# pairlab/SlotFormer

Hardware: AMD Instinct MI355X
Metric: rollout frames/sec at B=32, 128x128, 7 slots, 6+50 steps (SAVi-encode + SlotFormer rollout) (higher is better)
Workload: dtype f32 storage; matmul/conv on split-bf16 MFMA (bf16x3: hi*hi+hi*lo+lo*hi, f32 accumulate)

## Files before the change

### slotformer_amd/csrc/engine.hip

```cpp
#include "../../include/slotformer_hip.h"
#include "sf_internal.h"
#include <map>
#include <vector>
#include "layer_fused.h"
#include "slot_chain.h"
#include <stdlib.h>

namespace {

inline size_t pad256(size_t nfloat) { return ((nfloat * sizeof(float)) + 255) & ~(size_t)255; }

struct Bump {
  char* p;
  size_t left;
  bool ok = true;
  size_t used = 0;
  float* take(size_t nfloat) {
    const size_t bytes = pad256(nfloat);
    if (bytes > left) {
      ok = false;
      return nullptr;
    }
    float* r = p ? (float*)(p + used) : nullptr;
    used += bytes;
// ... 45 lines not shown
    } else {
      SF_TRY(sf_linear_ex(ws.x2, rd, w.lin1_w, w.lin1_b, w.norm2_g, w.norm2_b, eps, nullptr, rd, 0, ws.hid,
                          sf_rows(ffn), Mq, ffn, d, 1, st));
      SF_TRY(sf_linear_ex(ws.hid, sf_rows(ffn), w.lin2_w, w.lin2_b, nullptr, nullptr, eps, ws.x2, rd, 0, dst, rd,
                          Mq, d, ffn, 0, st));
    }
    *out = dst;
  } else {
    if (Lq != L) return sf_set_err(-1, "row pruning requires norm_first", __FILE__, __LINE__);
    int fused = 1;
    if (sf_get_precision() >= 1 && !plain_gemms(sf_thread_opts()))
      fused = sf_qkv_attn_ex(x, nullptr, nullptr, eps, w.in_proj_w, w.in_proj_b, ws.att, B, L, L, d, heads, st);
    if (fused < 0 || fused > 1) return fused;
    if (fused == 1) {
      SF_TRY(sf_linear_ex(x, rd, w.in_proj_w, w.in_proj_b, nullptr, nullptr, eps, nullptr, rd, 0, ws.qkv,
                          sf_rows(3 * d), M, 3 * d, d, 0, st));
      SF_TRY(sf_mha_ex(ws.qkv, ws.att, B, L, L, d, heads, st));
    }
    SF_TRY(sf_linear_ex(ws.att, rd, w.out_proj_w, w.out_proj_b, nullptr, nullptr, eps, x, rd, 0, ws.y, rd, M, d,
                        d, 0, st));
    SF_TRY(sf_layernorm_ex(ws.y, rd, w.norm1_g, w.norm1_b, ws.x2, rd, M, d, eps, st));
    SF_TRY(sf_linear_ex(ws.x2, rd, w.lin1_w, w.lin1_b, nullptr, nullptr, eps, nullptr, rd, 0, ws.hid,
                        sf_rows(ffn), M, ffn, d, 1, st));
    SF_TRY(sf_linear_ex(ws.hid, sf_rows(ffn), w.lin2_w, w.lin2_b, nullptr, nullptr, eps, ws.x2, rd, 0, ws.y, rd,
                        M, d, ffn, 0, st));
    SF_TRY(sf_layernorm_ex(ws.y, rd, w.norm2_g, w.norm2_b, x, rd, M, d, eps, st));
    *out = x;
  }
  return 0;
}

int check_layers(const sf_tfm_layer* l, int n) {
  if (n > 0 && !l) return -1;
  for (int i = 0; i < n; ++i) {
    const sf_tfm_layer& w = l[i];
    if (!w.norm1_g || !w.norm1_b || !w.in_proj_w || !w.in_proj_b || !w.out_proj_w || !w.out_proj_b ||
        !w.norm2_g || !w.norm2_b || !w.lin1_w || !w.lin1_b || !w.lin2_w || !w.lin2_b)
      return -1;
  }
  return 0;
}

void step_window(const sf_rollouter* m, int s, int& nf, int& f0) {
  nf = (m->single_step && s + 1 < m->window_len) ? s + 1 : m->window_len;
  f0 = m->single_step ? s + 1 - nf : s;
}

struct RolloutPlan {
  enum Path { GENERIC, LONG_WINDOW, FUSED_ROWS, FUSED_RING } path = GENERIC;
  int tok_layers = 0;
  enum Attn { HEAD_PAIRS, ALL_HEADS, ROW_TILES } attn = HEAD_PAIRS;
  enum Ffn { CHUNK_PARTS, TILE, TILE_QKV } ffn = CHUNK_PARTS;
  bool seam = false;
  bool fused() const { return path == FUSED_ROWS || path == FUSED_RING; }
};

RolloutPlan plan_rollout(const sf_rollouter* m, int B, const SfThreadOpts& o) {
  RolloutPlan p;
  if (!m || !m->layers) return p;
  const int N = m->num_slots, W = m->window_len, Lmax = W * N, nl = m->num_layers, d = m->d_model;
  bool packed = true, tok_packed = nl >= 2;
  for (int l = 0; l < nl; ++l) {
    const sf_tfm_layer& w = m->layers[l];
    packed = packed && w.lin1_packed && w.lin2_packed && w.attn_in_packed && w.attn_out_packed;
    if (l + 1 < nl) tok_packed = tok_packed && w.tok_packed;
  }
  const int precision = o.precision >= 0 ? o.precision : sf_get_precision();
  const bool fusable = packed && !plain_gemms(o) && precision >= 1 && m->norm_first;
  const bool tok_on = tok_packed && (o.layer_tok > 0 || (o.layer_tok == 0 && sf_get_layer_tok() != 0));
  if (fusable && sf_layer_fused_ok(d, m->num_heads, m->ffn_dim, Lmax)) {
    p.path = (m->in_proj_packed && m->out_proj_packed && sf_step_boundary_ok(d, m->slot_size)) ? RolloutPlan::FUSED_RING
                                                                                               : RolloutPlan::FUSED_ROWS;
    bool tok = tok_on;
    for (int nf = m->single_step ? 1 : W; nf <= W && tok; ++nf) tok = sf_layer_tok_ok(nf * N);
    p.tok_layers = tok ? nl - 1 : 0;
    p.attn = (o.attn_rows == 128 || tok) ? RolloutPlan::ROW_TILES : (o.attn_heads == 8 ? RolloutPlan::ALL_HEADS : RolloutPlan::HEAD_PAIRS);
    if (p.attn != RolloutPlan::HEAD_PAIRS && o.ffn_tile >= 1)
      p.ffn = (p.attn == RolloutPlan::ROW_TILES && o.ffn_tile == 2) ? RolloutPlan::TILE_QKV : RolloutPlan::TILE;
    const int cus = o.cus > 0 && o.cus < 160 ? o.cus : 160;
    p.seam = p.path == RolloutPlan::FUSED_RING && p.attn == RolloutPlan::HEAD_PAIRS &&
             (o.seam >= 0 ? o.seam != 0 : sf_get_seam_fused() != 0) && sf_seam_blocks(B, N) <= cus;
  } else if (fusable && sf_layer_fused_ok(d, m->num_heads, m->ffn_dim, 1) && Lmax > 64 && sf_ffn_tiles(B * Lmax) <= 1024) {
    p.path = RolloutPlan::LONG_WINDOW;
    if (tok_on && Lmax <= 96 && !m->single_step && sf_layer_tok_ok(Lmax)) p.tok_layers = nl - 1;
  }
  return p;
}

struct RolloutWs {
  float* x;
  TfmWs tw;
  float* apb;
  float* xpb;
  float *xa, *xb2;
  int* counters;
  unsigned* seam_flags;
  float* ring;
  float* planes;
};

bool rollout_ws_take(Bump& bp, RolloutWs& w, const sf_rollouter* m, int B) {
  const size_t M = (size_t)B * m->window_len * m->num_slots, d = m->d_model;
  w.x = bp.take(M * d);
  tfm_ws_take(bp, w.tw, (int)M, (int)d, m->ffn_dim);
  w.apb = bp.take(8 * M * d);
  w.xpb = bp.take(4 * M * d);
  w.xa = bp.take(M * d);
  w.xb2 = bp.take(M * d);
  w.counters = (int*)bp.take(1024);
  w.seam_flags = (unsigned*)bp.take(1024);
  w.ring = bp.take((size_t)B * (m->window_len + 1) * m->num_slots * d);
  w.planes = bp.take(sf_attn_rows_plane_bytes(B) / 4);
  return bp.ok;
}

}

extern "C" {

size_t sf_rollout_workspace_bytes(const sf_rollouter* m, int B) {
  if (!m || B <= 0) return 0;
  Bump bp{nullptr, ~(size_t)0};
  RolloutWs w;
  rollout_ws_take(bp, w, m, B);
  return bp.used;
}

__global__ void spin_kernel(long long ticks) {
  const long long t0 = wall_clock64();
  while (wall_clock64() - t0 < ticks) __builtin_amdgcn_s_sleep(16);
}
extern "C" int sf_debug_spin(int us, void* stream) {
  SF_REQUIRE(us > 0 && us <= 100000, "sf_debug_spin: 1..100000 microseconds");
  hipLaunchKernelGGL(spin_kernel, dim3(1), dim3(64), 0, (hipStream_t)stream, (long long)us * 100);
// ... 22 lines not shown
}

__global__ void zero_f32_kernel(float* a, float* b, long long n) {
  const long long i = 4 * ((long long)blockIdx.x * blockDim.x + threadIdx.x);
  if (i >= n) return;
  const bool vec = i + 4 <= n && ((((unsigned long long)(a + i)) | ((unsigned long long)(b + i))) & 15ull) == 0;
  if (vec) {
    *(float4*)(a + i) = float4{0.f, 0.f, 0.f, 0.f};
    *(float4*)(b + i) = float4{0.f, 0.f, 0.f, 0.f};
  } else {
    for (long long j = i; j < n && j < i + 4; ++j) {
      a[j] = 0.f;
      b[j] = 0.f;
    }
  }
}

__global__ void zero_words_kernel(unsigned* a, unsigned* b) {
  unsigned* p = blockIdx.x == 0 ? a : b;
  if (p) p[threadIdx.x] = 0u;
}

int sf_rollout_f32(const sf_rollouter* m, float* slots, int B, int T_total, int pred_len, void* ws,
                   size_t ws_bytes, void* stream) {
  SF_REQUIRE(m && slots && ws, "null pointer");
  SF_REQUIRE(B >= 1 && pred_len >= 0, "bad batch / pred_len");
  SF_REQUIRE(m->num_slots >= 1 && m->slot_size > 0 && (m->slot_size % 4) == 0 && m->d_model > 0 &&
                 (m->d_model % 4) == 0 && m->ffn_dim > 0 && (m->ffn_dim % 4) == 0 && m->num_layers >= 1 &&
                 m->window_len >= 1, "bad rollouter shape");
  SF_REQUIRE(m->in_proj_w && m->in_proj_b && m->out_proj_w && m->out_proj_b && m->pe_tok, "null weight");
  SF_REQUIRE(check_layers(m->layers, m->num_layers) == 0, "null transformer-layer weight");
  const int n_in = m->single_step ? 1 : m->window_len;
  SF_REQUIRE(T_total >= n_in + pred_len, "slots buffer shorter than burn-in + pred_len");
  SF_REQUIRE(ws_bytes >= sf_rollout_workspace_bytes(m, B), "workspace too small");
  hipStream_t st = (hipStream_t)stream;
  const int N = m->num_slots, C = m->slot_size, d = m->d_model, W = m->window_len, nl = m->num_layers;
  const float eps = 1e-5f;
  Bump bp{(char*)ws, ws_bytes};
  RolloutWs w;
  if (!rollout_ws_take(bp, w, m, B)) return sf_set_err(-1, "workspace too small", __FILE__, __LINE__);
  const RolloutPlan p = plan_rollout(m, B, sf_thread_opts());
  const bool ring_in = p.path == RolloutPlan::FUSED_RING;
  const bool long_ffn = p.path == RolloutPlan::LONG_WINDOW;
  const int np = p.attn == RolloutPlan::HEAD_PAIRS ? 4 : 1;
  const int RF = W + 1;
  const long long bs = (long long)T_total * N * C;
  if (ring_in) {
    SF_TRY(sf_ring_init_ex(m->out_proj_packed, m->out_proj_b, m->in_proj_packed, m->in_proj_b, slots, bs, n_in, w.ring, RF, N, B, st));
  }
  if (p.fused() || long_ffn) {
    SF_REQUIRE(sf_ffn_tiles(B * W * N) <= 1024, "batch too large for the fused-layer tile counters");
    hipLaunchKernelGGL(zero_words_kernel, dim3(2), dim3(1024), 0, st, (unsigned*)w.counters, p.seam ? w.seam_flags : nullptr);
    SF_CHECK_LAUNCH();
    if (p.attn == RolloutPlan::ROW_TILES) {
      const long long nfl = (long long)(sf_attn_rows_plane_bytes(B) / 4), half = nfl / 2;
      hipLaunchKernelGGL(zero_f32_kernel, dim3((unsigned)(((half + 3) / 4 + 255) / 256)), dim3(256), 0, st, w.planes, w.planes + half, half);
      SF_CHECK_LAUNCH();
    }
  }
  float* apb2 = w.apb + (size_t)4 * B * W * N * d;
  float* ap0 = w.apb;
  bool attn0_done = false;
  for (int s = 0; s < pred_len; ++s) {
    int nf, f0;
    step_window(m, s, nf, f0);
    const int L = nf * N, pe_off = (W - nf) * N;
    const float* pe = m->pe_tok + (long long)pe_off * d;
    float* cin = nullptr;
    if (!ring_in) {
      SfRowMap pmap = sf_rows(d);
      pmap.base = (long long)pe_off * d;
      SF_TRY(sf_linear_ex(slots, sf_rows_batched(C, L, bs, (long long)f0 * N * C), m->in_proj_w, m->in_proj_b,
                          nullptr, nullptr, 0.f, m->pe_tok, pmap, L, w.x, sf_rows(d), B * L, d, C, 0, st));
      cin = w.x;
    }
    int l = 0;
    while (l < p.tok_layers) {
      const int nlt = (p.tok_layers - l) < 8 ? (p.tok_layers - l) : 8;
      float* xo = (cin == w.xa) ? w.xb2 : w.xa;
      if (ring_in)
        SF_TRY(sf_layer_tok_ex(l == 0 ? 1 : 0, cin, w.ring, RF, N, f0, pe, m->layers + l, nlt, eps, xo, B, L, st));
      else
        SF_TRY(sf_layer_tok_ex(0, cin, nullptr, 1, 1, 0, nullptr, m->layers + l, nlt, eps, xo, B, L, st));
      cin = xo;
      l += nlt;
    }
    if (!p.fused()) {
      int Lc = L;
      for (; l < nl; ++l) {
        const int Lq = (l == nl - 1 && m->norm_first) ? N : Lc;
        SF_TRY(tfm_layer(m->layers[l], cin, w.tw, B, Lc, Lq, d, m->num_heads, m->ffn_dim, m->norm_first, st, &cin,
                         long_ffn ? w.xpb : nullptr, long_ffn ? w.counters : nullptr));
        Lc = Lq;
      }
      const SfRowMap lastmap = (Lc == N) ? sf_rows(d) : sf_rows_batched(d, N, (long long)Lc * d, (long long)(Lc - N) * d);
      SF_TRY(sf_linear_ex(cin, lastmap, m->out_proj_w, m->out_proj_b, nullptr, nullptr, 0.f, nullptr, sf_rows(C), 0,
                          slots, sf_rows_batched(C, N, bs, (long long)(n_in + s) * N * C), B * N, C, d, 0, st));
      continue;
    }
    bool parts_in = false;
    float* parked = nullptr;
    for (; l < nl; ++l) {
      const sf_tfm_layer& lw = m->layers[l];
      const bool lastl = (l == nl - 1);
      const int Lq = lastl ? N : L;
      const long long pst = (long long)B * Lq * d;
      float* xo = (cin == w.xa) ? w.xb2 : w.xa;
      float* ap = (l == 0) ? ap0 : w.apb;
      if (parked) {
        ap = parked;
        SF_TRY(sf_attn_core_ex(lw, ap, w.planes, B, L, Lq, st));
      } else if (p.attn == RolloutPlan::ROW_TILES) {
        if (l == 0 && ring_in)
          SF_TRY(sf_attn_rows_ex(2, w.ring, (long long)RF * N * d, 0, pe, f0, RF, N, lw, eps, ap, w.planes, B, L, Lq, st));
        else if (parts_in)
          SF_TRY(sf_attn_rows_ex(1, w.xpb, (long long)L * d, (long long)B * L * d, nullptr, 0, 1, 1, lw, eps, ap, w.planes, B, L, Lq, st));
        else
          SF_TRY(sf_attn_rows_ex(0, cin, (long long)L * d, 0, nullptr, 0, 1, 1, lw, eps, ap, w.planes, B, L, Lq, st));
      } else if (p.attn == RolloutPlan::ALL_HEADS) {
        if (l == 0 && ring_in)
          SF_TRY(sf_attn_all_ring_ex(w.ring, RF, N, f0, pe, lw, eps, ap, B, L, Lq, st));
        else if (parts_in)
          SF_TRY(sf_attn_all_parts_ex(w.xpb, (long long)B * L * d, lw, eps, ap, B, L, Lq, st));
        else
          SF_TRY(sf_attn_all_ex(cin, lw, eps, ap, B, L, Lq, st));
      } else if (l == 0 && ring_in) {
        if (!attn0_done) SF_TRY(sf_attn_oproj_ring_ex(w.ring, RF, N, f0, pe, lw, eps, ap, pst, B, L, Lq, st));
      } else if (parts_in) {
        SF_TRY(sf_attn_oproj_parts_ex(w.xpb, (long long)B * L * d, lw, eps, ap, pst, B, L, Lq, st));
      } else {
        SF_TRY(sf_attn_oproj_ex(cin, lw, eps, ap, pst, B, L, Lq, st));
      }
      if (!lastl) {
        if (p.ffn == RolloutPlan::TILE_QKV) {
          float* park = (ap == w.apb) ? apb2 : w.apb;
          SF_TRY(sf_ffn_qkv_tile_ex(ap, lw, m->layers[l + 1], eps, park, w.planes, B, L, (l + 1 == nl - 1) ? N : L, m->ffn_dim, st));
          parked = park;
          cin = nullptr;
        } else if (p.ffn == RolloutPlan::TILE) {
// ... 790 lines not shown
```

### slotformer_amd/csrc/layer_fused.h

```cpp
#pragma once
#include "../../include/slotformer_hip.h"
#include "sf_internal.h"

int sf_pred_step_ex(const float* prev, const sf_tfm_layer* layers, int nlayers, int heads, int ffn, int norm_first, const void* const* packed,
                    const float* lstm_b_ih, const float* lstm_b_hh, const float* proj_b, int hidden, float* lstm_h, float* lstm_c,
                    float* out, int B, int N, int D, float eps, hipStream_t st);

int sf_attn_oproj_ex(const float* xin, const sf_tfm_layer& w, float eps, float* ap, long long ap_stride, int B, int L,
                     int Lq, hipStream_t st);
int sf_attn_oproj_parts_ex(const float* xparts, long long xparts_stride, const sf_tfm_layer& w, float eps, float* ap,
                           long long ap_stride, int B, int L, int Lq, hipStream_t st);
int sf_ffn_parts_ex(const float* ap, long long ap_stride, const sf_tfm_layer& w, float eps, float* xp, long long xp_stride, int M,
                    int ffn, hipStream_t st, int np = 4);
int sf_attn_all_ex(const float* xin, const sf_tfm_layer& w, float eps, float* x2, int B, int L, int Lq, hipStream_t st);
int sf_attn_all_parts_ex(const float* xparts, long long xparts_stride, const sf_tfm_layer& w, float eps, float* x2, int B, int L,
                         int Lq, hipStream_t st);
int sf_attn_all_ring_ex(const float* ring, int ring_frames, int nslots, int f0, const float* pe, const sf_tfm_layer& w, float eps,
                        float* x2, int B, int L, int Lq, hipStream_t st);
int sf_attn_core_ex(const sf_tfm_layer& w, float* x2, void* planes, int B, int L, int Lq, hipStream_t st);
int sf_ffn_qkv_tile_ex(const float* x2, const sf_tfm_layer& w, const sf_tfm_layer& wn, float eps, float* xpark, void* planes, int B, int L, int Lq,
                       int ffn, hipStream_t st);
int sf_ffn_tile_ex(const float* x2, const sf_tfm_layer& w, float eps, float* y, int M, int ffn, hipStream_t st);
bool sf_layer_tok_ok(int L);
int sf_layer_tok_vpw(int L);
int sf_layer_tok_ex(int mode, const float* xin, const float* ring, int ring_frames, int nslots, int f0, const float* pe, const sf_tfm_layer* layers, int nl,
                    float eps, float* y, int B, int L, hipStream_t st);
size_t sf_attn_rows_plane_bytes(int B);
int sf_attn_rows_ex(int mode, const float* xin, long long x_batch_stride, long long xparts_stride, const float* pe, int f0,
                    int ring_frames, int nslots, const sf_tfm_layer& w, float eps, float* x2, void* planes, int B, int L, int Lq,
                    hipStream_t st);
int sf_attn_oproj_ring_ex(const float* ring, int ring_frames, int nslots, int f0, const float* pe, const sf_tfm_layer& w,
                          float eps, float* ap, long long ap_stride, int B, int L, int Lq, hipStream_t st);
bool sf_step_boundary_ok(int d, int slot_size);
int sf_ffn_partial_ex(const float* ap, long long ap_stride, const sf_tfm_layer& w, float eps, float* xp,
                      long long xp_stride, float* xout, int* counters, int M, int ffn, hipStream_t st, int np = 4);
int sf_ffn_tiles(int M);
int sf_ring_init_ex(const void* wout_packed, const float* b_out, const void* win_packed, const float* b_in, float* slots,
                    long long slots_bs, int n_frames, float* ring, int ring_frames, int nslots, int B, hipStream_t st);
int sf_ffn_boundary_ex(const float* ap, long long ap_stride, const sf_tfm_layer& w, float eps, float* xp, long long xp_stride,
                       int* counters, int ffn, const void* wout_packed, const float* b_out, const void* win_packed,
                       const float* b_in, float* slots, long long slots_bs, int frame, float* ring, int ring_frames, int nslots,
                       int B, hipStream_t st, int np = 4);
int sf_seam_ex(const float* ap_ffn, long long pst_ffn, const sf_tfm_layer& wl, float eps, float* xp, long long xp_stride,
               int* counters, int ffn, const void* wout_packed, const float* b_out, const void* win_packed, const float* b_in,
               float* slots, long long slots_bs, int frame, float* ring, int ring_frames, int nslots, int B,
               const sf_tfm_layer& w0, int f0_next, const float* pe, float* ap_attn, long long pst_attn, int L, int Lq,
               unsigned* seam_flags, unsigned epoch, hipStream_t st);
int sf_seam_blocks(int B, int nslots);
bool sf_seam_window_ok(int L, int nslots);
```

### slotformer_amd/csrc/layer_tok.hip

```cpp
#include "../../include/slotformer_hip.h"
#include "sf_internal.h"
#include "layer_fused.h"
#include <stdlib.h>

typedef float f32x16 __attribute__((ext_vector_type(16)));
typedef float f32x4 __attribute__((ext_vector_type(4)));
typedef __bf16 bf16x4 __attribute__((ext_vector_type(4)));
typedef __bf16 bf16x8 __attribute__((ext_vector_type(8)));

namespace {
constexpr int LT_NT = 256, LT_D = 256, LT_F = 1024, LT_NH = 8, LT_TOK = 128, LT_MAXL = 8;
constexpr int LT_STAGE = 32 * 1024, LT_RING = 3;
constexpr int LT_NST_ATT = 4 * LT_NH, LT_NST = LT_NST_ATT + 2 * (LT_F / 32);
constexpr int LT_KV = LT_RING * LT_STAGE;
constexpr int LT_VT = LT_KV + 16 * 1024;
constexpr int LT_PAR = LT_KV + 32 * 1024;
constexpr int P_LN1G = 0, P_LN1B = 256, P_BQKV = 512, P_BO = 1280, P_LN2G = 1536, P_LN2B = 1792, P_B1 = 2048, P_B2 = 3072, P_N = 3328;
constexpr size_t LT_LDS = (size_t)LT_PAR + (size_t)P_N * 4;
constexpr size_t LT_BLOB = (size_t)LT_NST * LT_STAGE + (size_t)P_N * 4;
static_assert(LT_LDS <= 160 * 1024, "LDS budget");

struct LtArgs {
  const float* x;
  const float* ring;
  const float* pe;
  float* y;
  const char* blob[LT_MAXL];
  float eps;
  int nl, B, L, vpw, RF, N, f0, dbg_ts;
};

__device__ __forceinline__ bf16x8 cat8(bf16x4 a, bf16x4 b) { return __builtin_shufflevector(a, b, 0, 1, 2, 3, 4, 5, 6, 7); }
__device__ __forceinline__ void split8(const f32x4 a, const f32x4 b, bf16x8& hi, bf16x8& lo) {
  const bf16x4 h0 = __builtin_convertvector(a, bf16x4), h1 = __builtin_convertvector(b, bf16x4);
  const bf16x4 l0 = __builtin_convertvector(a - __builtin_convertvector(h0, f32x4), bf16x4);
  const bf16x4 l1 = __builtin_convertvector(b - __builtin_convertvector(h1, f32x4), bf16x4);
  hi = cat8(h0, h1);
  lo = cat8(l0, l1);
}
__device__ __forceinline__ f32x4 quad(const f32x16& a, int g) { return f32x4{a[4 * g], a[4 * g + 1], a[4 * g + 2], a[4 * g + 3]}; }
__device__ __forceinline__ float lt_xother(float v, int h) {
#ifdef LT_SHFL
  return __shfl_xor(v, 32, 64);
#endif
  const unsigned u = __builtin_bit_cast(unsigned, v);
  const auto r = __builtin_amdgcn_permlane32_swap(u, u, false, false);
  return __builtin_bit_cast(float, h ? r[0] : r[1]);
}
__device__ __forceinline__ float lt_xmax(float v, int h) { return fmaxf(v, lt_xother(v, h)); }
__device__ __forceinline__ float lt_xsum(float v, int h) {
  const float o = lt_xother(v, h);
  return h ? o + v : v + o;
}

struct LtRing {
  const char* rd;
  const char* src;
  char* dst;
};
__device__ __forceinline__ void lt_dma_now(const LtRing& R, int f) {
  __builtin_amdgcn_global_load_lds((const void __attribute__((address_space(1)))*)(R.src + f * 1024),
                                   (void __attribute__((address_space(3)))*)(R.dst + f * 1024), 16, 0, 0);
}
__device__ __forceinline__ void lt_dma(const LtRing& R, int f) {
#if defined(LT_NODMA) || defined(LT_BURST)
  return;
#endif
#ifndef LT_NOIMMOFF
  const void __attribute__((address_space(1)))* s = (const void __attribute__((address_space(1)))*)(R.src + (f >> 2) * 4096);
  void __attribute__((address_space(3)))* d = (void __attribute__((address_space(3)))*)(R.dst + (f >> 2) * 4096);
  switch (f & 3) {
    case 0: __builtin_amdgcn_global_load_lds(s, d, 16, 0, 0); break;
    case 1: __builtin_amdgcn_global_load_lds(s, d, 16, 1024, 0); break;
    case 2: __builtin_amdgcn_global_load_lds(s, d, 16, 2048, 0); break;
    default: __builtin_amdgcn_global_load_lds(s, d, 16, 3072, 0); break;
  }
#else
  __builtin_amdgcn_global_load_lds((const void __attribute__((address_space(1)))*)(R.src + f * 1024),
                                   (void __attribute__((address_space(3)))*)(R.dst + f * 1024), 16, 0, 0);
#endif
}
#define LT_MFMA(a, b, c) __builtin_amdgcn_mfma_f32_32x32x16_bf16(a, b, c, 0, 0, 0)
// ... 212 lines not shown
      hd = 7; kind = 3;
    } else {
      const int tq = st - 3;
      kind = tq & 3;
      hd = 1 + (tq >> 2) - (kind == 3 ? 1 : 0);
    }
    slice = kind == 3;
    ld = LT_D;
    if (!slice) {
      W = win; r0 = (kind == 0 ? 0 : kind == 1 ? 256 : 512) + 32 * hd;
    } else {
      W = wout; c0 = 32 * hd;
    }
  } else {
    const int ff = st - LT_NST_ATT;
    int hb;
    if (ff == 0) {
      slice = false; hb = 0;
    } else if (ff == 63) {
      slice = true; hb = 31;
    } else if (ff & 1) {
      slice = false; hb = (ff + 1) >> 1;
    } else {
      slice = true; hb = (ff >> 1) - 1;
    }
    if (!slice) {
      W = w1; ld = LT_D; r0 = 32 * hb;
    } else {
      W = w2; ld = LT_F; c0 = 32 * hb;
    }
  }
  if (!slice) {
    const int vk = f >> 1;
    c0 = 32 * (vk >> 1);
    s = vk & 1;
  } else {
    r0 = 32 * (f >> 2);
    s = (f >> 1) & 1;
  }
  const float* src = W + (long long)(r0 + i) * ld + c0 + 4 * h;
  union {
    __bf16 b[8];
    uint4 u;
  } o;
#pragma unroll
  for (int j = 0; j < 8; ++j) {
    const float v = src[8 * (2 * s + (j >> 2)) + (j & 3)];
    const __bf16 hi = (__bf16)v;
    o.b[j] = pl ? (__bf16)(v - (float)hi) : hi;
  }
  out[idx] = o.u;
}

__device__ long long lt_ts[16];
#define LTS(i) do { if (A.dbg_ts && blockIdx.x == 0 && threadIdx.x == 0) lt_ts[i] = wall_clock64(); } while (0)

template <int MODE>
__global__ __launch_bounds__(LT_NT) void layer_tok_kernel(LtArgs A) {
  extern __shared__ __attribute__((aligned(16))) char smem[];
  float* P = (float*)(smem + LT_PAR);
  const int t = threadIdx.x, lane = t & 63;
  const int wave = __builtin_amdgcn_readfirstlane(t >> 6);
  const int n = lane & 31, h = lane >> 5;
  const int L = A.L;
  const int v0 = blockIdx.x * A.vpw;
  const int nvalid = min(A.vpw, A.B - v0) * L;
  const int tl = wave * 32 + n;
  const int te = min(tl, nvalid - 1);
  const int vl = te / L, tok = te - vl * L;
  const long long row = (long long)(v0 + vl) * L + tok;
  LTS(0);
  f32x16 X[8];
  if constexpr (MODE == 0) {
    const float* xr = A.x + row * LT_D + 4 * h;
#pragma unroll
    for (int ob = 0; ob < 8; ++ob)
#pragma unroll
      for (int g = 0; g < 4; ++g) {
        const f32x4 v = *(const f32x4*)(xr + 32 * ob + 8 * g);
#pragma unroll
        for (int q = 0; q < 4; ++q) X[ob][4 * g + q] = v[q];
      }
  } else {
    const int fr = tok / A.N, sl = tok - fr * A.N;
    const float* rr = A.ring + (((long long)(v0 + vl) * A.RF + (A.f0 + fr) % A.RF) * A.N + sl) * LT_D + 4 * h;
    const float* pr = A.pe + (long long)tok * LT_D + 4 * h;
#pragma unroll
    for (int ob = 0; ob < 8; ++ob)
#pragma unroll
      for (int g = 0; g < 4; ++g) {
        const f32x4 v = *(const f32x4*)(rr + 32 * ob + 8 * g);
#pragma unroll
        for (int q = 0; q < 4; ++q) X[ob][4 * g + q] = v[q];
      }
    __builtin_amdgcn_sched_barrier(0);
#pragma unroll
    for (int ob = 0; ob < 8; ++ob) {
#pragma unroll
      for (int g = 0; g < 4; ++g) {
        const f32x4 v = *(const f32x4*)(pr + 32 * ob + 8 * g);
#pragma unroll
        for (int q = 0; q < 4; ++q) X[ob][4 * g + q] += v[q];
      }
      __builtin_amdgcn_sched_barrier(0);
    }
  }
  const unsigned wlane = (unsigned)(wave * 8 * 1024 + lane * 16);
  char* const wdst = smem + (wave * 8) * 1024;
  int cur = 0;
  int cs = -2;
// ... 25 lines not shown
    const long long c0 = __builtin_readcyclecounter();
    if (c_last) c_work += c0 - c_last;
#endif
#ifdef LT_NODMA
    asm volatile("s_waitcnt vmcnt(0)" ::: "memory");
#else
    asm volatile("s_waitcnt vmcnt(8)" ::: "memory");
#endif
    asm volatile("s_waitcnt lgkmcnt(0)" ::: "memory");
#ifdef LT_STAMPS
    const long long c1 = __builtin_readcyclecounter();
#endif
#ifndef LT_NOBAR
    __builtin_amdgcn_s_barrier();
#endif
    asm volatile("" ::: "memory");
#ifdef LT_STAMPS
    c_last = __builtin_readcyclecounter();
    c_wait += c1 - c0;
    c_bar += c_last - c1;
#endif
    const int nb = cur == 0 ? 2 : cur - 1;
    LtRing R{smem + cur * LT_STAGE + lane * 16, stage_src(), wdst + nb * LT_STAGE};
#ifdef LT_BURST
#pragma unroll
    for (int f = 0; f < 8; ++f) lt_dma_now(R, f);
#endif
    cur = cur == 2 ? 0 : cur + 1;
    return R;
  };
  const int wf = min(wave * 32, nvalid - 1);
  const int kb0 = ((wf / L) * L) >> 5;
  const int d0 = 32 * kb0 + 4 * h - vl * L;
  const char* pb;
  {
    unsigned pbo = (unsigned)(LT_PAR + 16 * h);
    asm volatile("" : "+v"(pbo));
    pb = smem + pbo;
  }
  char* const kwr = smem + LT_KV + wave * 1024 + lane * 16;
  char* const vwr = smem + LT_VT + wave * 4096 + lane * 16;
  const char* krd[3];
  const char* vrd[3];
#pragma unroll
  for (int kbi = 0; kbi < 3; ++kbi) {
    const int kb = min(kb0 + kbi, 3);
    krd[kbi] = smem + LT_KV + kb * 1024 + lane * 16;
    vrd[kbi] = smem + LT_VT + kb * 4096 + lane * 16;
  }
  const float qscale = 0.2550348616841918f;
  constexpr float NEG = -3.0e38f;
  LTS(1);

#pragma unroll 1
  for (int l = 0; l < A.nl; ++l) {
    cs = 0;
    base_cur = A.blob[l];
    last_layer = l + 1 >= A.nl;
    base_nxt = A.blob[last_layer ? l : l + 1];
    __syncthreads();
    {
      const float* vsrc = (const float*)(A.blob[l] + (size_t)LT_NST * LT_STAGE);
      for (int i = t; i < P_N / 4; i += LT_NT) *(f32x4*)(P + 4 * i) = *(const f32x4*)(vsrc + 4 * i);
    }
    __syncthreads();
    if (l == 0) LTS(2);
    bf16x8 xh[16], xl[16];
    lt_layernorm<P_LN1G, P_LN1B>(X, pb, h, A.eps, xh, xl);
    lt_add_vec<P_BO>(X, pb);
    if (l == 0) LTS(3);
    f32x16 qa, ka, va, S[3], O;
    bf16x8 qh[2], ql[2], ph[3][2], pl[3][2], oh[2], ol[2];
    float mx0 = NEG, mx1 = NEG, mx = 0.f, sm = 0.f, rinv = 0.f;
    auto zero16 = [](f32x16& a) {
#pragma unroll
      for (int r = 0; r < 16; ++r) a[r] = 0.f;
    };
    int hq = 0;
    auto mask_chunk = [&](int c) {
      const int kbi = c >> 1;
#pragma unroll
      for (int rr = 0; rr < 8; ++rr) {
        const int r = 8 * (c & 1) + rr;
        const bool ok = (unsigned)(d0 + 32 * kbi + 8 * (r >> 2) + (r & 3)) < (unsigned)L;
        const float v = ok ? S[kbi][r] : NEG;
        S[kbi][r] = v;
        if (rr & 1) mx1 = fmaxf(mx1, v); else mx0 = fmaxf(mx0, v);
      }
    };
    auto exp_chunk = [&](int c) {
      const int kbi = c >> 1;
      float s0 = 0.f, s1 = 0.f;
#pragma unroll
      for (int rr = 0; rr < 8; ++rr) {
        const int r = 8 * (c & 1) + rr;
#ifdef LT_EXPF
        const float e = __expf((S[kbi][r] - mx) * 0.6931471805599453f);
#else
        const float e = __builtin_amdgcn_exp2f(S[kbi][r] - mx);
#endif
        S[kbi][r] = e;
        if (rr & 1) s1 += e; else s0 += e;
      }
      sm += s0 + s1;
    };
    auto psplit_chunk = [&](int c) { split8(quad(S[c >> 1], 2 * (c & 1)), quad(S[c >> 1], 2 * (c & 1) + 1), ph[c >> 1][c & 1], pl[c >> 1][c & 1]); };
    auto kconv = [&](int s) {
      const float* bk = (const float*)pb + P_BQKV + 256 + 32 * hq;
// ... 87 lines not shown
      lt_row_product<true, 5>(R, xh, xl, va, [&](int g) {
        if (g < 2) kconv(g);
        else if (g < 4) qconv(g - 2);
      });
      vconv(0);
      vconv(1);
    }
#pragma unroll 1
    for (hq = 1; hq < LT_NH; ++hq) {
      {
        const LtRing R = stage_begin();
        scores();
          lt_row_product<false, 6>(R, xh, xl, qa, sideD);
      }
      {
        const LtRing R = stage_begin();
          lt_row_product<false, 6>(R, xh, xl, ka, sideA);
        pv();
      }
      {
        const LtRing R = stage_begin();
          lt_row_product<true, 5>(R, xh, xl, va, [&](int g) {
          if (g < 2) kconv(g);
          else if (g < 4) qconv(g - 2);
          else if (g < 6) oconv(g - 4);
        });
      }
      {
        const LtRing R = stage_begin();
        lt_kslice_product<5>(R, oh, ol, X, [&](int g) {
          if (g < 2) vconv(g);
        });
      }
    }
    asm volatile("s_waitcnt lgkmcnt(0)" ::: "memory");
    __builtin_amdgcn_s_barrier();
    asm volatile("" ::: "memory");
    scores();
#pragma unroll
    for (int g = 0; g < 8; ++g) sideD(g);
#pragma unroll
    for (int g = 0; g < 6; ++g) sideA(g);
    pv();
    oconv(0);
    oconv(1);
    {
      const LtRing R = stage_begin();
      lt_kslice_product<0>(R, oh, ol, X, LtNoSide{});
    }
    if (l == 0) LTS(4);
#ifdef LT_STAMPS
    if (l == 0 && blockIdx.x == 0 && threadIdx.x == 0) { lt_ts[8] = c_wait; lt_ts[9] = c_bar; lt_ts[10] = c_work; }
#endif
    lt_layernorm<P_LN2G, P_LN2B>(X, pb, h, A.eps, xh, xl);
    lt_add_vec<P_B2>(X, pb);
    if (l == 0) LTS(5);
    f32x16 Ha, Hb;
    bf16x8 hh[2], hl[2];
    f32x4 b1q[4];
    auto b1_load = [&](int blk) {
      const float* b1 = (const float*)pb + P_B1 + 32 * blk;
#pragma unroll
      for (int g = 0; g < 4; ++g) b1q[g] = *(const f32x4*)(b1 + 8 * g);
    };
    auto hconv = [&](const f32x16& Hx, int s) {
      const f32x4 z4 = {0.f, 0.f, 0.f, 0.f};
      const f32x4 u0 = __builtin_elementwise_max(quad(Hx, 2 * s) + b1q[2 * s], z4);
      const f32x4 u1 = __builtin_elementwise_max(quad(Hx, 2 * s + 1) + b1q[2 * s + 1], z4);
      split8(u0, u1, hh[s], hl[s]);
    };
    auto ffn_step = [&](f32x16& Hn, const f32x16& Hp, int j) {
      {
        const LtRing R = stage_begin();
        lt_row_product<false, 4>(R, xh, xl, Hn, [&](int g) {
          if (g >= 1 && g < 3) hconv(Hp, g - 1);
        });
        asm volatile("" : "+v"(hh[0]), "+v"(hh[1]), "+v"(hl[0]), "+v"(hl[1]));
      }
      {
        const LtRing R = stage_begin();
        b1_load(j);
        lt_kslice_product<0>(R, hh, hl, X, LtNoSide{});
      }
    };
    {
      const LtRing R = stage_begin();
      b1_load(0);
      lt_row_product<false, 0>(R, xh, xl, Ha, LtNoSide{});
    }
    ffn_step(Hb, Ha, 1);
#pragma unroll 1
    for (int j = 2; j < LT_F / 32; j += 2) {
      ffn_step(Ha, Hb, j);
      ffn_step(Hb, Ha, j + 1);
    }
    hconv(Hb, 0);
    hconv(Hb, 1);
    {
      const LtRing R = stage_begin();
      lt_kslice_product<0>(R, hh, hl, X, LtNoSide{});
    }
    if (l == 0) LTS(6);
#ifdef LT_STAMPS
    if (l == 0 && blockIdx.x == 0 && threadIdx.x == 0) { lt_ts[11] = c_wait; lt_ts[12] = c_bar; lt_ts[13] = c_work; }
#endif
  }
  asm volatile("s_waitcnt vmcnt(0)" ::: "memory");
  if (tl < nvalid) {
    float* yr = A.y + row * LT_D + 4 * h;
#pragma unroll
    for (int ob = 0; ob < 8; ++ob)
#pragma unroll
      for (int g = 0; g < 4; ++g) *(f32x4*)(yr + 32 * ob + 8 * g) = quad(X[ob], g);
  }
  LTS(7);
}

extern "C" int sf_debug_read_ts_layer_tok(long long* out16) {
  hipError_t e = hipMemcpyFromSymbol(out16, HIP_SYMBOL(lt_ts), sizeof(long long) * 16);
  return e == hipSuccess ? 0 : (int)e;
}

extern "C" size_t sf_layer_tok_packed_bytes(void) { return LT_BLOB; }

extern "C" int sf_pack_layer_tok_weights(const sf_tfm_layer* w, void* packed, int d_model, int num_heads, int ffn, void* stream) {
  SF_REQUIRE(w && packed, "sf_pack_layer_tok_weights: null pointer");
  SF_REQUIRE(w->in_proj_w && w->out_proj_w && w->lin1_w && w->lin2_w && w->norm1_g && w->norm1_b && w->in_proj_b && w->out_proj_b && w->norm2_g &&
                 w->norm2_b && w->lin1_b && w->lin2_b, "sf_pack_layer_tok_weights: null weight");
  SF_REQUIRE(d_model == LT_D && num_heads == LT_NH && ffn == LT_F, "sf_pack_layer_tok_weights: d_model 256, 8 heads, ffn 1024 only");
  hipStream_t st = (hipStream_t)stream;
  const int total = LT_NST * 32 * 64;
  hipLaunchKernelGGL(pack_layer_tok_kernel, dim3((total + 255) / 256), dim3(256), 0, st, w->in_proj_w, w->out_proj_w, w->lin1_w, w->lin2_w, (uint4*)packed);
  SF_CHECK_LAUNCH();
  float* vec = (float*)((char*)packed + (size_t)LT_NST * LT_STAGE);
  const struct {
    const float* src;
    int off, n;
  } parts[8] = {{w->norm1_g, P_LN1G, 256}, {w->norm1_b, P_LN1B, 256}, {w->in_proj_b, P_BQKV, 768}, {w->out_proj_b, P_BO, 256},
                {w->norm2_g, P_LN2G, 256}, {w->norm2_b, P_LN2B, 256}, {w->lin1_b, P_B1, 1024},   {w->lin2_b, P_B2, 256}};
  for (const auto& p : parts) {
    const hipError_t e = hipMemcpyAsync(vec + p.off, p.src, (size_t)p.n * 4, hipMemcpyDeviceToDevice, st);
    if (e != hipSuccess) return sf_set_err((int)e, hipGetErrorString(e), __FILE__, __LINE__);
  }
  return 0;
}

int sf_layer_tok_vpw(int L) {
  if (L < 1 || L > 96) return 0;
  for (int vpw = LT_TOK / L; vpw >= 1; --vpw) {
    const int nvalid = vpw * L;
    bool ok = true;
    for (int w = 0; w < 4 && ok; ++w) {
      const int wf = w * 32 < nvalid ? w * 32 : nvalid - 1, wl = w * 32 + 31 < nvalid ? w * 32 + 31 : nvalid - 1;
      const int kb0 = ((wf / L) * L) >> 5, kb1 = (((wl / L) * L) + L - 1) >> 5;
      ok = kb1 - kb0 + 1 <= 3;
    }
    if (ok) return vpw;
  }
  return 0;
}
bool sf_layer_tok_ok(int L) { return sf_layer_tok_vpw(L) > 0; }

int sf_layer_tok_ex(int mode, const float* xin, const float* ring, int ring_frames, int nslots, int f0, const float* pe, const sf_tfm_layer* layers, int nl,
                    float eps, float* y, int B, int L, hipStream_t st) {
  bool ok = layers && nl >= 1 && nl <= LT_MAXL && sf_layer_tok_ok(L) && B >= 1 && y && (mode == 0 ? xin != nullptr : (ring && pe && nslots >= 1 && ring_frames >= 1));
  for (int l = 0; ok && l < nl; ++l) ok = layers[l].tok_packed != nullptr;
  if (!ok)
    return sf_set_err(-1, "invalid argument: the token-stationary layers need sf_pack_layer_tok_weights fragments, 1..8 layers and 1 <= L <= 96 rows per video", __FILE__, __LINE__);
  static const int dbg = sf_dbg("lt");
  LtArgs A;
  A.x = xin; A.ring = ring; A.pe = pe; A.y = y;
  for (int l = 0; l < LT_MAXL; ++l) A.blob[l] = (const char*)layers[l < nl ? l : nl - 1].tok_packed;
  A.eps = eps; A.nl = nl; A.B = B; A.L = L; A.vpw = sf_layer_tok_vpw(L); A.RF = ring_frames; A.N = nslots; A.f0 = f0; A.dbg_ts = dbg;
  const int nwg = (B + A.vpw - 1) / A.vpw;
  const double flops = nl * ((double)B * L * (2.0 * LT_D * (3 * LT_D + LT_D + 2 * LT_F)) + (double)B * LT_NH * 4.0 * L * L * 32);
  if (mode == 0) {
    SF_TRY(sf_ensure_dyn_lds((const void*)layer_tok_kernel<0>, LT_LDS));
    sf_prof_begin(SF_K_LAYER_TOK, st, flops);
    hipLaunchKernelGGL(layer_tok_kernel<0>, dim3(nwg), dim3(LT_NT), LT_LDS, st, A);
  } else {
    SF_TRY(sf_ensure_dyn_lds((const void*)layer_tok_kernel<1>, LT_LDS));
    sf_prof_begin(SF_K_LAYER_TOK, st, flops);
    hipLaunchKernelGGL(layer_tok_kernel<1>, dim3(nwg), dim3(LT_NT), LT_LDS, st, A);
  }
  sf_prof_end(SF_K_LAYER_TOK, st);
  SF_CHECK_LAUNCH();
  return 0;
}

extern "C" int sf_layer_tok_block_f32(const sf_tfm_layer* w, int nl, const float* x, float* y, int B, int L, void* stream) {
  SF_REQUIRE(w && x && y && B > 0 && nl >= 1 && nl <= LT_MAXL, "sf_layer_tok_block_f32: null pointer / empty problem / more than 8 layers");
  SF_REQUIRE(sf_get_precision() == 1, "sf_layer_tok_block_f32: split-bf16 mode only");
  return sf_layer_tok_ex(0, x, nullptr, 1, 1, 0, nullptr, w, nl, 1e-5f, y, B, L, (hipStream_t)stream);
}
```

Measured before the change: 668,700.

## Fold last transformer layer and slot boundary projections into token-stationary kernel

Extends the token-stationary layer kernel so the final transformer layer (attention plus LN2, FFN, residual) and the out-projection and in-projection at the step boundary run inside the same launch, only for the last N slot rows. The kernel writes predicted slots and the next ring entry directly, so the per-step launches of the separate fused last-layer path and its plane zeroing are skipped. The cost is a longer kernel with FFN weights streamed per workgroup from registers and LDS. Only one wave-group of 32 rows does the tail work, which may be underutilized.

```diff
diff --git a/slotformer_amd/csrc/engine.hip b/slotformer_amd/csrc/engine.hip
--- a/slotformer_amd/csrc/engine.hip
+++ b/slotformer_amd/csrc/engine.hip
@@ -121,6 +121,7 @@
   enum Attn { HEAD_PAIRS, ALL_HEADS, ROW_TILES } attn = HEAD_PAIRS;
   enum Ffn { CHUNK_PARTS, TILE, TILE_QKV } ffn = CHUNK_PARTS;
   bool seam = false;
+  bool fold = false;
   bool fused() const { return path == FUSED_ROWS || path == FUSED_RING; }
 };
 
@@ -149,6 +150,8 @@
     const int cus = o.cus > 0 && o.cus < 160 ? o.cus : 160;
     p.seam = p.path == RolloutPlan::FUSED_RING && p.attn == RolloutPlan::HEAD_PAIRS &&
              (o.seam >= 0 ? o.seam != 0 : sf_get_seam_fused() != 0) && sf_seam_blocks(B, N) <= cus;
+    p.fold = p.path == RolloutPlan::FUSED_RING && p.tok_layers == nl - 1 && p.tok_layers > 0 && m->layers[nl - 1].tok_packed && !m->single_step &&
+             m->ffn_dim == 1024 && sf_layer_tok_fold_ok(Lmax, N);
   } else if (fusable && sf_layer_fused_ok(d, m->num_heads, m->ffn_dim, 1) && Lmax > 64 && sf_ffn_tiles(B * Lmax) <= 1024) {
     p.path = RolloutPlan::LONG_WINDOW;
     if (tok_on && Lmax <= 96 && !m->single_step && sf_layer_tok_ok(Lmax)) p.tok_layers = nl - 1;
@@ -277,7 +280,7 @@
     SF_REQUIRE(sf_ffn_tiles(B * W * N) <= 1024, "batch too large for the fused-layer tile counters");
     hipLaunchKernelGGL(zero_words_kernel, dim3(2), dim3(1024), 0, st, (unsigned*)w.counters, p.seam ? w.seam_flags : nullptr);
     SF_CHECK_LAUNCH();
-    if (p.attn == RolloutPlan::ROW_TILES) {
+    if (p.attn == RolloutPlan::ROW_TILES && !p.fold) {
       const long long nfl = (long long)(sf_attn_rows_plane_bytes(B) / 4), half = nfl / 2;
       hipLaunchKernelGGL(zero_f32_kernel, dim3((unsigned)(((half + 3) / 4 + 255) / 256)), dim3(256), 0, st, w.planes, w.planes + half, half);
       SF_CHECK_LAUNCH();
@@ -303,13 +306,18 @@
     while (l < p.tok_layers) {
       const int nlt = (p.tok_layers - l) < 8 ? (p.tok_layers - l) : 8;
       float* xo = (cin == w.xa) ? w.xb2 : w.xa;
-      if (ring_in)
-        SF_TRY(sf_layer_tok_ex(l == 0 ? 1 : 0, cin, w.ring, RF, N, f0, pe, m->layers + l, nlt, eps, xo, B, L, st));
-      else
+      if (ring_in) {
+        const SfTokFold fold{m->layers + nl - 1, m->ffn_dim, m->out_proj_packed, m->in_proj_packed, m->out_proj_b, m->in_proj_b,
+                             slots, bs, n_in + s, w.ring, RF};
+        const bool fold_here = p.fold && l + nlt == p.tok_layers;
+        SF_TRY(sf_layer_tok_ex(l == 0 ? 1 : 0, cin, w.ring, RF, N, f0, pe, m->layers + l, nlt, eps, xo, B, L, st, fold_here ? &fold : nullptr));
+      } else {
         SF_TRY(sf_layer_tok_ex(0, cin, nullptr, 1, 1, 0, nullptr, m->layers + l, nlt, eps, xo, B, L, st));
+      }
       cin = xo;
       l += nlt;
     }
+    if (p.fold) continue;
     if (!p.fused()) {
       int Lc = L;
       for (; l < nl; ++l) {
diff --git a/slotformer_amd/csrc/layer_fused.h b/slotformer_amd/csrc/layer_fused.h
--- a/slotformer_amd/csrc/layer_fused.h
+++ b/slotformer_amd/csrc/layer_fused.h
@@ -23,8 +23,20 @@
 int sf_ffn_tile_ex(const float* x2, const sf_tfm_layer& w, float eps, float* y, int M, int ffn, hipStream_t st);
 bool sf_layer_tok_ok(int L);
 int sf_layer_tok_vpw(int L);
+struct SfTokFold {
+  const sf_tfm_layer* last;
+  int ffn;
+  const void *wout_packed, *win_packed;
+  const float *b_out, *b_in;
+  float* slots;
+  long long slots_bs;
+  int frame;
+  float* ring;
+  int ring_frames;
+};
+bool sf_layer_tok_fold_ok(int L, int nslots);
 int sf_layer_tok_ex(int mode, const float* xin, const float* ring, int ring_frames, int nslots, int f0, const float* pe, const sf_tfm_layer* layers, int nl,
-                    float eps, float* y, int B, int L, hipStream_t st);
+                    float eps, float* y, int B, int L, hipStream_t st, const SfTokFold* fold = nullptr);
 size_t sf_attn_rows_plane_bytes(int B);
 int sf_attn_rows_ex(int mode, const float* xin, long long x_batch_stride, long long xparts_stride, const float* pe, int f0,
                     int ring_frames, int nslots, const sf_tfm_layer& w, float eps, float* x2, void* planes, int B, int L, int Lq,
diff --git a/slotformer_amd/csrc/layer_tok.hip b/slotformer_amd/csrc/layer_tok.hip
--- a/slotformer_amd/csrc/layer_tok.hip
+++ b/slotformer_amd/csrc/layer_tok.hip
@@ -25,9 +25,14 @@
   const float* ring;
   const float* pe;
   float* y;
-  const char* blob[LT_MAXL];
+  const char* blob[LT_MAXL + 1];
   float eps;
   int nl, B, L, vpw, RF, N, f0, dbg_ts;
+  const uint4 *w1p, *w2p, *wout_p, *win_p;
+  const float *ln2g, *ln2b, *b1, *b2, *b_out, *b_in;
+  float* slots;
+  float* ring_out;
+  long long slots_bs, slots_off, ring_bs, ring_off;
 };
 
 __device__ __forceinline__ bf16x8 cat8(bf16x4 a, bf16x4 b) { return __builtin_shufflevector(a, b, 0, 1, 2, 3, 4, 5, 6, 7); }
@@ -346,10 +351,202 @@
   out[idx] = o.u;
 }
 
+constexpr int PF_AP = LT_D + 8, PF_XP = LT_D + 4, PF_C = 128, PF_PP = PF_C + 8;
+constexpr size_t PF_AH = 0, PF_AL = PF_AH + 32 * PF_AP * 2, PF_HH = PF_AL + 32 * PF_AP * 2, PF_HL = PF_HH + 32 * PF_AP * 2;
+constexpr size_t PF_X2 = PF_HL + 32 * PF_AP * 2, PF_END = PF_X2 + (size_t)32 * PF_XP * 4;
+static_assert(PF_END <= (size_t)LT_PAR && (size_t)2 * 32 * PF_PP * 2 <= 2 * 32 * PF_AP * 2, "folded last layer: LDS budget");
+
+__device__ __forceinline__ void lt_split4(__bf16* hp, __bf16* lp, int off, f32x4 v) {
+  const bf16x4 hi = __builtin_convertvector(v, bf16x4);
+  const bf16x4 lo = __builtin_convertvector(v - __builtin_convertvector(hi, f32x4), bf16x4);
+  *(bf16x4*)(hp + off) = hi;
+  *(bf16x4*)(lp + off) = lo;
+}
+__device__ __forceinline__ f32x16 lt_frag_product(const bf16x8 (&wf)[16][2], const __bf16* bh, const __bf16* bl) {
+  f32x16 a0, a1;
+#pragma unroll
+  for (int r = 0; r < 16; ++r) a0[r] = a1[r] = 0.f;
+#pragma unroll
+  for (int ks = 0; ks < 16; ks += 2) {
+    const bf16x8 xh0 = *(const bf16x8*)(bh + ks * 16), xl0 = *(const bf16x8*)(bl + ks * 16);
+    const bf16x8 xh1 = *(const bf16x8*)(bh + ks * 16 + 16), xl1 = *(const bf16x8*)(bl + ks * 16 + 16);
+    a0 = LT_MFMA(wf[ks][0], xl0, a0);
+    a1 = LT_MFMA(wf[ks + 1][0], xl1, a1);
+    a0 = LT_MFMA(wf[ks][1], xh0, a0);
+    a1 = LT_MFMA(wf[ks + 1][1], xh1, a1);
+    a0 = LT_MFMA(wf[ks][0], xh0, a0);
+    a1 = LT_MFMA(wf[ks + 1][0], xh1, a1);
+  }
+  return a0 + a1;
+}
+
+__device__ __forceinline__ void lt_fold_tail(const LtArgs& A, char* smem, const f32x16 (&X)[8], int wave, int lane, int tl, int te, int nvalid) {
+#pragma clang fp contract(off)
+  __bf16* Ah = (__bf16*)(smem + PF_AH);
+  __bf16* Al = (__bf16*)(smem + PF_AL);
+  __bf16* Hh = (__bf16*)(smem + PF_HH);
+  __bf16* Hl = (__bf16*)(smem + PF_HL);
+  float* X2 = (float*)(smem + PF_X2);
+  const int n = lane & 31, h = lane >> 5, L = A.L, N = A.N;
+  const int v0 = blockIdx.x * A.vpw, nq = (nvalid / L) * N;
+  {
+    const int vl = te / L, tok = te - vl * L;
+    if (tl < nvalid && tok >= L - N) {
+      float* xr = X2 + (vl * N + tok - (L - N)) * PF_XP + 4 * h;
+#pragma unroll
+      for (int ob = 0; ob < 8; ++ob)
+#pragma unroll
+        for (int g = 0; g < 4; ++g) *(f32x4*)(xr + 32 * ob + 8 * g) = quad(X[ob], g);
+    }
+  }
+  __syncthreads();
+  {
+    const f32x4 g = *(const f32x4*)(A.ln2g + 4 * lane), be = *(const f32x4*)(A.ln2b + 4 * lane);
+#pragma unroll
+    for (int i = 0; i < 8; ++i) {
+      const int r = wave + 4 * i;
+      const f32x4 x2 = *(const f32x4*)(X2 + min(r, nq - 1) * PF_XP + 4 * lane);
+      const float mean = sf_sum64((x2[0] + x2[1]) + (x2[2] + x2[3])) * (1.0f / LT_D);
+      const f32x4 dv = x2 - mean;
+      const float rstd = 1.0f / sqrtf(sf_sum64((dv[0] * dv[0] + dv[1] * dv[1]) + (dv[2] * dv[2] + dv[3] * dv[3])) * (1.0f / LT_D) + A.eps);
+      lt_split4(Ah, Al, r * PF_AP + 4 * lane, (x2 - mean) * rstd * g + be);
+    }
+  }
+  __syncthreads();
+  const int ao = n * PF_AP + 8 * h;
+  const int rn = min(n, nq - 1);
+  bf16x8 wf[2][16][2];
+  auto load = [&](int j, bf16x8 (&w)[16][2]) {
+    const int c = j >> 2, wb = wave + 4 * (j & 1);
+    const uint4* base = (((j >> 1) & 1) ? A.w2p : A.w1p) + ((long long)(c * 16) * 8 + wb) * 128 + lane;
+#pragma unroll
+    for (int ks = 0; ks < 16; ++ks)
+#pragma unroll
+      for (int pl = 0; pl < 2; ++pl) w[ks][pl] = __builtin_bit_cast(bf16x8, base[(ks * 8) * 128 + pl * 64]);
+  };
+  f32x16 Hacc[2], Y[2];
+  load(0, wf[0]);
+#pragma unroll
+  for (int j = 0; j < 16; ++j) {
+    if (j + 1 < 16) load(j + 1, wf[(j + 1) & 1]);
+    const int c = j >> 2, jb = j & 1, wb = wave + 4 * jb;
+    if (((j >> 1) & 1) == 0) {
+      Hacc[jb] = lt_frag_product(wf[j & 1], Ah + ao, Al + ao);
+      if (jb == 1) {
+        __syncthreads();
+#pragma unroll
+        for (int b = 0; b < 2; ++b) {
+          const int hb = wave + 4 * b;
+#pragma unroll
+          for (int g = 0; g < 4; ++g) {
+            const f32x4 bv = *(const f32x4*)(A.b1 + c * 256 + hb * 32 + 4 * h + 8 * g);
+            f32x4 hv;
+#pragma unroll
+            for (int q = 0; q < 4; ++q) hv[q] = fmaxf(Hacc[b][4 * g + q] + bv[q], 0.f);
+            lt_split4(Hh, Hl, n * PF_AP + hb * 32 + 4 * h + 8 * g, hv);
+          }
+        }
+        __syncthreads();
+      }
+    } else {
+      const f32x16 p = lt_frag_product(wf[j & 1], Hh + ao, Hl + ao);
+      if (c == 0) {
+#pragma unroll
+        for (int g = 0; g < 4; ++g) {
+          const int col = wb * 32 + 4 * h + 8 * g;
+          const f32x4 r = *(const f32x4*)(X2 + rn * PF_XP + col) + *(const f32x4*)(A.b2 + col);
+#pragma unroll
+          for (int q = 0; q < 4; ++q) Y[jb][4 * g + q] = p[4 * g + q] + r[q];
+        }
+      } else {
+#pragma unroll
+        for (int r = 0; r < 16; ++r) Y[jb][r] = Y[jb][r] + p[r];
+      }
+    }
+  }
+#pragma unroll
+  for (int b = 0; b < 2; ++b)
+#pragma unroll
+    for (int g = 0; g < 4; ++g) lt_split4(Ah, Al, n * PF_AP + (wave + 4 * b) * 32 + 4 * h + 8 * g, quad(Y[b], g));
+  __syncthreads();
+  const bool st_ok = n < nq;
+  const long long vb = v0 + n / N, sn = n - (n / N) * N;
+  __bf16* Ph = Hh;
+  __bf16* Pl = Hh + 32 * PF_PP;
+  {
+    bf16x8 wo[16][2];
+#pragma unroll
+    for (int ks = 0; ks < 16; ++ks)
+#pragma unroll
+      for (int pl = 0; pl < 2; ++pl) wo[ks][pl] = __builtin_bit_cast(bf16x8, A.wout_p[(((long long)ks * 4 + wave) * 2 + pl) * 64 + lane]);
+    f32x16 a0, a1;
+#pragma unroll
+    for (int r = 0; r < 16; ++r) a0[r] = a1[r] = 0.f;
+#pragma unroll
+    for (int k = 0; k < 8; ++k) {
+      const bf16x8 xh0 = *(const bf16x8*)(Ah + ao + k * 16), xl0 = *(const bf16x8*)(Al + ao + k * 16);
+      const bf16x8 xh1 = *(const bf16x8*)(Ah + ao + 128 + k * 16), xl1 = *(const bf16x8*)(Al + ao + 128 + k * 16);
+      a0 = LT_MFMA(wo[k][0], xl0, a0);
+      a1 = LT_MFMA(wo[8 + k][0], xl1, a1);
+      a0 = LT_MFMA(wo[k][1], xh0, a0);
+      a1 = LT_MFMA(wo[8 + k][1], xh1, a1);
+      a0 = LT_MFMA(wo[k][0], xh0, a0);
+      a1 = LT_MFMA(wo[8 + k][0], xh1, a1);
+    }
+#pragma unroll
+    for (int g = 0; g < 4; ++g) {
+      const int col = wave * 32 + 4 * h + 8 * g;
+      const f32x4 bo = *(const f32x4*)(A.b_out + col);
+      f32x4 v;
+#pragma unroll
+      for (int q = 0; q < 4; ++q) v[q] = a0[4 * g + q] + a1[4 * g + q] + bo[q];
+      lt_split4(Ph, Pl, n * PF_PP + col, v);
+      if (st_ok) *(f32x4*)(A.slots + vb * A.slots_bs + A.slots_off + sn * PF_C + col) = v;
+    }
+  }
+  __syncthreads();
+  {
+    bf16x8 wi[2][8][2];
+#pragma unroll
+    for (int b = 0; b < 2; ++b)
+#pragma unroll
+      for (int k = 0; k < 8; ++k)
+#pragma unroll
+        for (int pl = 0; pl < 2; ++pl) wi[b][k][pl] = __builtin_bit_cast(bf16x8, A.win_p[(((long long)k * 8 + wave + 4 * b) * 2 + pl) * 64 + lane]);
+    f32x16 a[2];
+#pragma unroll
+    for (int r = 0; r < 16; ++r) a[0][r] = a[1][r] = 0.f;
+    const int po = n * PF_PP + 8 * h;
+#pragma unroll
+    for (int k = 0; k < 8; ++k) {
+      const bf16x8 xh = *(const bf16x8*)(Ph + po + k * 16), xl = *(const bf16x8*)(Pl + po + k * 16);
+#pragma unroll
+      for (int b = 0; b < 2; ++b) a[b] = LT_MFMA(wi[b][k][0], xl, a[b]);
+#pragma unroll
+      for (int b = 0; b < 2; ++b) a[b] = LT_MFMA(wi[b][k][1], xh, a[b]);
+#pragma unroll
+      for (int b = 0; b < 2; ++b) a[b] = LT_MFMA(wi[b][k][0], xh, a[b]);
+    }
+    if (st_ok) {
+#pragma unroll
+      for (int b = 0; b < 2; ++b)
+#pragma unroll
+        for (int g = 0; g < 4; ++g) {
+          const int col = (wave + 4 * b) * 32 + 4 * h + 8 * g;
+          const f32x4 bi = *(const f32x4*)(A.b_in + col);
+          f32x4 v;
+#pragma unroll
+          for (int q = 0; q < 4; ++q) v[q] = a[b][4 * g + q] + bi[q];
+          *(f32x4*)(A.ring_out + vb * A.ring_bs + A.ring_off + sn * LT_D + col) = v;
+        }
+    }
+  }
+}
+
 __device__ long long lt_ts[16];
 #define LTS(i) do { if (A.dbg_ts && blockIdx.x == 0 && threadIdx.x == 0) lt_ts[i] = wall_clock64(); } while (0)
 
-template <int MODE>
+template <int MODE, bool FOLD>
 __global__ __launch_bounds__(LT_NT) void layer_tok_kernel(LtArgs A) {
   extern __shared__ __attribute__((aligned(16))) char smem[];
   float* P = (float*)(smem + LT_PAR);
@@ -481,8 +678,14 @@
   constexpr float NEG = -3.0e38f;
   LTS(1);
 
+#ifdef LT_STAMPS
+  long long c_fold = 0;
+#endif
 #pragma unroll 1
   for (int l = 0; l < A.nl; ++l) {
+#ifdef LT_STAMPS
+    if (FOLD && l + 1 == A.nl) c_fold = __builtin_readcyclecounter();
+#endif
     cs = 0;
     base_cur = A.blob[l];
     last_layer = l + 1 >= A.nl;
@@ -676,6 +879,9 @@
 #ifdef LT_STAMPS
     if (l == 0 && blockIdx.x == 0 && threadIdx.x == 0) { lt_ts[8] = c_wait; lt_ts[9] = c_bar; lt_ts[10] = c_work; }
 #endif
+    if constexpr (FOLD) {
+      if (l + 1 == A.nl) break;
+    }
     lt_layernorm<P_LN2G, P_LN2B>(X, pb, h, A.eps, xh, xl);
     lt_add_vec<P_B2>(X, pb);
     if (l == 0) LTS(5);
@@ -730,6 +936,22 @@
 #endif
   }
   asm volatile("s_waitcnt vmcnt(0)" ::: "memory");
+  if constexpr (FOLD) {
+#ifdef LT_STAMPS
+    const long long cf0 = __builtin_readcyclecounter();
+#endif
+    __syncthreads();
+    lt_fold_tail(A, smem, X, wave, lane, tl, te, nvalid);
+    LTS(7);
+#ifdef LT_STAMPS
+    if (A.dbg_ts && blockIdx.x == 0 && threadIdx.x == 0) {
+      const long long cf1 = __builtin_readcyclecounter();
+      lt_ts[14] = cf1 - cf0;
+      lt_ts[15] = cf1 - c_fold;
+    }
+#endif
+    return;
+  }
   if (tl < nvalid) {
     float* yr = A.y + row * LT_D + 4 * h;
 #pragma unroll
@@ -784,28 +1006,61 @@
   return 0;
 }
 bool sf_layer_tok_ok(int L) { return sf_layer_tok_vpw(L) > 0; }
+bool sf_layer_tok_fold_ok(int L, int nslots) {
+  const int vpw = sf_layer_tok_vpw(L);
+  return vpw > 0 && nslots >= 1 && nslots <= L && vpw * nslots <= 32;
+}
 
 int sf_layer_tok_ex(int mode, const float* xin, const float* ring, int ring_frames, int nslots, int f0, const float* pe, const sf_tfm_layer* layers, int nl,
-                    float eps, float* y, int B, int L, hipStream_t st) {
+                    float eps, float* y, int B, int L, hipStream_t st, const SfTokFold* fold) {
   bool ok = layers && nl >= 1 && nl <= LT_MAXL && sf_layer_tok_ok(L) && B >= 1 && y && (mode == 0 ? xin != nullptr : (ring && pe && nslots >= 1 && ring_frames >= 1));
   for (int l = 0; ok && l < nl; ++l) ok = layers[l].tok_packed != nullptr;
   if (!ok)
     return sf_set_err(-1, "invalid argument: the token-stationary layers need sf_pack_layer_tok_weights fragments, 1..8 layers and 1 <= L <= 96 rows per video", __FILE__, __LINE__);
+  if (fold) {
+    const sf_tfm_layer* w = fold->last;
+    const bool fok = w && w->tok_packed && w->lin1_packed && w->lin2_packed && w->norm2_g && w->norm2_b && w->lin1_b && w->lin2_b &&
+                     fold->ffn == LT_F && fold->wout_packed && fold->win_packed && fold->b_out && fold->b_in && fold->slots && fold->frame >= 0 &&
+                     fold->ring && fold->ring_frames >= 1 &&
+                     sf_layer_tok_fold_ok(L, nslots);
+    if (!fok)
+      return sf_set_err(-1, "invalid argument: the folded last layer needs packed FFN / boundary weights and at most 32 rows per workgroup", __FILE__, __LINE__);
+  }
   static const int dbg = sf_dbg("lt");
-  LtArgs A;
+  LtArgs A{};
   A.x = xin; A.ring = ring; A.pe = pe; A.y = y;
-  for (int l = 0; l < LT_MAXL; ++l) A.blob[l] = (const char*)layers[l < nl ? l : nl - 1].tok_packed;
+  for (int l = 0; l <= LT_MAXL; ++l) A.blob[l] = (const char*)layers[l < nl ? l : nl - 1].tok_packed;
   A.eps = eps; A.nl = nl; A.B = B; A.L = L; A.vpw = sf_layer_tok_vpw(L); A.RF = ring_frames; A.N = nslots; A.f0 = f0; A.dbg_ts = dbg;
   const int nwg = (B + A.vpw - 1) / A.vpw;
-  const double flops = nl * ((double)B * L * (2.0 * LT_D * (3 * LT_D + LT_D + 2 * LT_F)) + (double)B * LT_NH * 4.0 * L * L * 32);
-  if (mode == 0) {
-    SF_TRY(sf_ensure_dyn_lds((const void*)layer_tok_kernel<0>, LT_LDS));
+  double flops = nl * ((double)B * L * (2.0 * LT_D * (3 * LT_D + LT_D + 2 * LT_F)) + (double)B * LT_NH * 4.0 * L * L * 32);
+  if (fold) {
+    const sf_tfm_layer* w = fold->last;
+    A.blob[nl] = (const char*)w->tok_packed;
+    A.nl = nl + 1;
+    A.w1p = (const uint4*)w->lin1_packed; A.w2p = (const uint4*)w->lin2_packed;
+    A.wout_p = (const uint4*)fold->wout_packed; A.win_p = (const uint4*)fold->win_packed;
+    A.ln2g = w->norm2_g; A.ln2b = w->norm2_b; A.b1 = w->lin1_b; A.b2 = w->lin2_b; A.b_out = fold->b_out; A.b_in = fold->b_in;
+    A.slots = fold->slots; A.slots_bs = fold->slots_bs; A.slots_off = (long long)fold->frame * nslots * PF_C;
+    A.ring_out = fold->ring; A.ring_bs = (long long)fold->ring_frames * nslots * LT_D;
+    A.ring_off = (long long)(fold->frame % fold->ring_frames) * nslots * LT_D;
+    flops += (double)B * L * (2.0 * LT_D * 4 * LT_D) + (double)B * LT_NH * 4.0 * L * L * 32 + (double)B * nslots * (4.0 * LT_D * LT_F + 4.0 * LT_D * PF_C);
+  }
+  if (fold && mode == 0) {
+    SF_TRY(sf_ensure_dyn_lds((const void*)layer_tok_kernel<0, true>, LT_LDS));
     sf_prof_begin(SF_K_LAYER_TOK, st, flops);
-    hipLaunchKernelGGL(layer_tok_kernel<0>, dim3(nwg), dim3(LT_NT), LT_LDS, st, A);
+    hipLaunchKernelGGL((layer_tok_kernel<0, true>), dim3(nwg), dim3(LT_NT), LT_LDS, st, A);
+  } else if (fold) {
+    SF_TRY(sf_ensure_dyn_lds((const void*)layer_tok_kernel<1, true>, LT_LDS));
+    sf_prof_begin(SF_K_LAYER_TOK, st, flops);
+    hipLaunchKernelGGL((layer_tok_kernel<1, true>), dim3(nwg), dim3(LT_NT), LT_LDS, st, A);
+  } else if (mode == 0) {
+    SF_TRY(sf_ensure_dyn_lds((const void*)layer_tok_kernel<0, false>, LT_LDS));
+    sf_prof_begin(SF_K_LAYER_TOK, st, flops);
+    hipLaunchKernelGGL((layer_tok_kernel<0, false>), dim3(nwg), dim3(LT_NT), LT_LDS, st, A);
   } else {
-    SF_TRY(sf_ensure_dyn_lds((const void*)layer_tok_kernel<1>, LT_LDS));
+    SF_TRY(sf_ensure_dyn_lds((const void*)layer_tok_kernel<1, false>, LT_LDS));
     sf_prof_begin(SF_K_LAYER_TOK, st, flops);
-    hipLaunchKernelGGL(layer_tok_kernel<1>, dim3(nwg), dim3(LT_NT), LT_LDS, st, A);
+    hipLaunchKernelGGL((layer_tok_kernel<1, false>), dim3(nwg), dim3(LT_NT), LT_LDS, st, A);
   }
   sf_prof_end(SF_K_LAYER_TOK, st);
   SF_CHECK_LAUNCH();
```

New measurement: 674,900, median of 6. Within noise of the previous version (+0.9%).
